# dayae1204/WeCLIP-ViT-CoMer

Hardware: AMD Instinct MI355X
Metric: images/sec (train fwd+bwd) ViT-B/16 512x512 VOC (higher is better)
Workload: dtype f16 MFMA operands / f32 accumulate, f32 residual+softmax+LN, PAR f32 arithmetic on 16-bit fixed-point affinities (precision=fast); 1 GPU; WeCLIP VOC full train step (the reference's model: frozen CLIP ViT-B/16 + adapters + decoder + GradCAM/affinity/PAR pseudo-labels), batch 16/GPU at 512x512, K=2 classes/image (BASELINE configs[2] without the ViT-CoMer inserts, for which the reference has no code); global_batch=16, parallelism=dp1

## Files before the change

### include/weclip_hip.h

```cpp
#ifndef WECLIP_HIP_H
#define WECLIP_HIP_H
#include <stdint.h>
#ifdef __cplusplus
extern "C" {
#endif

int wc_version(void);
const char* wc_last_error(void);
int wc_device_count(void);
int wc_device_arch(int dev, char* buf, int buflen);

void wc_prof_enable(int stride);
void wc_prof_tag(const char* tag);
int wc_prof_report(char* buf, int cap);

int wc_par_affinity(const float* img, float* aff, int B, int H, int W,
                    const int* h_dilations, int n_dil, void* stream);
int wc_par_iterate(const float* aff, const float* masks_in, float* masks_out, int B, int C,
                   int H, int W, const int* h_dilations, int n_dil, void* stream);
int wc_par_forward(const float* img, const float* masks, float* out, float* tmp, float* aff_ws,
                   int B, int C, int H, int W, const int* h_dilations, int n_dil, int num_iter,
                   int group, void* stream);
int wc_par_forward_h(const float* img, const float* masks, float* out, float* tmp, float* aff_ws,
                   int B, int C, int H, int W, const int* h_dilations, int n_dil, int num_iter,
// ... 24 lines not shown
                const void* W2, int nseg, int M, int N, int K, long lda, long ldw, int batch,
                long sA, long sW, long sC, const float* bias, const float* resid, long ldr, long sR,
                float* C32,
                void* C16, void* C16lo, long ldc, int act, int round16, float scale,
                int scale_cols, float* P32, const float* aux, const int* rowmap, int rpg,
                long ldaux, const void* auxh, const float* cscale, long sCS, void* stream);

int wc_gemm_f16_grouped(const void* A0, const void* A1, const void* A2, const void* W0, const void* W1,
                        const void* W2, int nseg, int M, int N, int K, long lda, long ldw, int batch,
                        long sA, long sW, long sC, const float* bias, const float* resid, long ldr, long sR,
                        float* C32, void* C16, void* C16lo, long ldc, int act, int round16, float scale,
                        int scale_cols, float* P32, const float* aux, const int* rowmap, int rpg,
                        long ldaux, const void* auxh, const float* cscale, long sCS, int zdiv, long sA2, long sW2,
                        long sC2, long sB2, long sX2, void* stream);

int wc_gemm_row_supported(int M, int N, int K);
int wc_gemm_row_f16(const void* A, long lda, const void* W, long ldw, int M, int N, int K, const float* bias,
                    const float* cscale, int act, const float* aux, const void* auxh, long ldaux, const float* resid, long ldr,
                    float* C32, void* C16, float* P32, long ldc, long ldc16, const float* ln_g0, const float* ln_b0, void* ln_o0,
                    const float* ln_g1, const float* ln_b1, void* ln_o1, float eps, void* stream);

int wc_gemm_row_f16_grouped(const void* A, long lda, const void* W, long ldw, int M, int N, int K, const float* bias, int act,
                            const void* auxh, long ldaux, float* C32, void* C16, long ldc, long ldc16, int groups, long gA,
                            long gW, long gB, long gC, long gX, void* stream);

int wc_gemm_plan(int M, int N, int K, int nseg, int batch);
int wc_gemm_log_report(char* buf, int cap);
int wc_sum_slices(const float* part, float* out, int nslices, long n, float alpha, void* stream);

int wc_sum_slices_wb(const float* part, float* out_w, float* out_b, int nslices, int rows, int cols,
// ... 24 lines not shown

int wc_attn_fwd(const void* qkv, void* out, float* out32, float* lse, int B, int L, int H, int DH,
                void* stream);
int wc_attn_mean(const void* qkv, const float* lse, float* mean, int B, int L, int H, int DH,
                 void* stream);

int wc_patchify(const float* img, void* hi, void* lo, int B, int H, int W, int P, void* stream);
int wc_cls_rows(float* x, const float* cls, const float* pos0, int B, int L, int E, void* stream);

int wc_cam_head(const float* x2, const float* lnw, const float* lnb, const float* proj,
                const float* text, const int* text_idx, const int* n_text, const int* pair_img,
                const int* pair_cls, float logit_scale, float* partial, float* probs, float* df,
                int B, int P, int L, int E, int Ed, int Tmax, void* stream);
int wc_lnpost_bwd(const float* df, const float* x2, const float* lnw, float gs, const int* pair_img,
                  float* d32, void* dhi, void* dlo, int P, int L, int E, void* stream);
int wc_ln2_bwd_add(const float* da2, const float* dx2, const float* x1, const float* lnw, float gs,
                   const int* pair_img, void* g16, int P, int L, int E, void* stream);
int wc_attn_bwd_colsum(const void* qkv, const void* dO, const float* o32, const float* lse,
                       const int* pair_img, float* delta, float* u, float* dS0, float* P0, float* c,
                       int P, int L, int H, int DH, void* stream);
int wc_rowvec_matmul(const float* c, const float* W, float* out, float* ws, int P, int N, int E, float scale,
                     void* stream);
int wc_cam_map(const float* a32, const float* w, const int* pair_img, float* cam, int P, int L, int E,
               void* stream);

int wc_aff_weight(const float* const* h_maps, int nmaps, const float* wgt, const float* seg, float* W,
                  int B, int L, void* stream);
int wc_aff_seg_weights(const float* const* h_maps, int nmaps, const float* seg, float* diff, float* wgt,
                       int B, int L, void* stream);
int wc_matvec(const float* W, const float* X, const float* sin, const float* sout, const float* add,
// ... 215 lines not shown
```

### weclip-vit-comer_amd/csrc/gemm.hip

```cpp
#include "common.h"
#include <cstring>
#include <stdlib.h>

#include <map>
#include <string>
#include <vector>

struct GemmShapeRec { char key[96]; hipEvent_t e0, e1; double flop; };
static int g_shape_log = -1;
static std::vector<GemmShapeRec> g_shape_recs;
int shape_log_begin(void* stream) {
    if (g_shape_log < 0) g_shape_log = getenv("WECLIP_GEMM_LOG") ? atoi(getenv("WECLIP_GEMM_LOG")) : 0;
    if (!g_shape_log) return -1;
    GemmShapeRec r;
    r.key[0] = 0; r.flop = 0;
    hipEventCreate(&r.e0); hipEventCreate(&r.e1);
    hipEventRecord(r.e0, (hipStream_t)stream);
    g_shape_recs.push_back(r);
    return (int)g_shape_recs.size() - 1;
}
void shape_log_end(int idx, const char* kind, int M, int N, int K, int nseg, int batch, int plan, int act, void* stream) {
    if (idx < 0) return;
    GemmShapeRec& r = g_shape_recs[idx];
    snprintf(r.key, sizeof(r.key), "%s M=%d N=%d K=%d seg=%d batch=%d plan=%d act=%d", kind, M, N, K, nseg, batch, plan, act);
// ... 493 lines not shown
    const long gx = wc_cdiv(N, 256), gy = wc_cdiv(M, 256);
    if (!pp_mode || batch != 1 || (long)K * nseg < 2 * BK || gx * gy < pp_min_tiles) return 0;
    if ((long)M * lda * 2 >= (1L << 32) || (long)N * ldw * 2 >= (1L << 32)) return 0;
    const int n_cu = gemm_cu_count();
    const bool can_split = M % 256 != 0 && !row_mapped_aux;
    const bool split = can_split && wc_cdiv(gx * (gy - 1), n_cu) < wc_cdiv(gx * gy, n_cu);
    return split ? 2 : 1;
}

extern "C" int wc_gemm_plan(int M, int N, int K, int nseg, int batch) {
    return gemm_plan(M, N, K, nseg, batch, false);
}

struct GemmKernel { void (*fn)(GemmArgs); int threads; int lds; const char* name; };
#define GEMM_KERNEL(threads_, lds_, ...) {__VA_ARGS__, threads_, lds_, #__VA_ARGS__}
static const GemmKernel gemm_pp_kernels[4] = {
    GEMM_KERNEL(512, 10 * PP_SLOT, gemm_f16_pp_kernel<0, 10>), GEMM_KERNEL(512, 10 * PP_SLOT, gemm_f16_pp_kernel<1, 10>),
    GEMM_KERNEL(512, 8 * PP_SLOT, gemm_f16_pp_kernel<2, 8>), GEMM_KERNEL(512, 8 * PP_SLOT, gemm_f16_pp_kernel<3, 8>)};
static const GemmKernel gemm_skinny_kernels[4] = {
    GEMM_KERNEL(256, 0, gemm_skinny_kernel<0>), GEMM_KERNEL(256, 0, gemm_skinny_kernel<1>),
    GEMM_KERNEL(256, 0, gemm_skinny_kernel<2>), GEMM_KERNEL(256, 0, gemm_skinny_kernel<3>)};
static const GemmKernel gemm_tile_kernels[2][4] = {
    {GEMM_KERNEL(256, 2 * 2 * BM * BK * 2, gemm_f16_kernel<0, 2>), GEMM_KERNEL(256, 2 * 2 * BM * BK * 2, gemm_f16_kernel<1, 2>),
     GEMM_KERNEL(256, 2 * 2 * BM * BK * 2, gemm_f16_kernel<2, 2>), GEMM_KERNEL(256, 2 * 2 * BM * BK * 2, gemm_f16_kernel<3, 2>)},
    {GEMM_KERNEL(256, 4 * 2 * BM * BK * 2, gemm_f16_kernel<0, 4>), GEMM_KERNEL(256, 4 * 2 * BM * BK * 2, gemm_f16_kernel<1, 4>),
     GEMM_KERNEL(256, 4 * 2 * BM * BK * 2, gemm_f16_kernel<2, 4>), GEMM_KERNEL(256, 4 * 2 * BM * BK * 2, gemm_f16_kernel<3, 4>)}};
#undef GEMM_KERNEL

static bool gemm_reserve_lds(const GemmKernel* k, int n) {
    for (int i = 0; i < n; ++i)
        if (k[i].lds > 65536 &&
            hipFuncSetAttribute((const void*)k[i].fn, hipFuncAttributeMaxDynamicSharedMemorySize, k[i].lds) != hipSuccess)
            return false;
    return true;
}

static int gemm_launch(const GemmKernel& k, const char* family, dim3 grid, const GemmArgs& g, double flop, void* stream) {
    const int pr = wc_prof_begin(stream);
    hipLaunchKernelGGL(k.fn, grid, dim3(k.threads), k.lds, (hipStream_t)stream, g);
    wc_prof_end(pr, k.name, flop, stream);
    WC_LAUNCH_CHECK(family);
    return WC_OK;
}

static int gemm_dispatch(GemmArgs g, int batch, void* stream) {
    int M = g.M;
    const int N = g.N, K = g.K, act = g.act;
    const int ek = ((act == 6 || act == 7) ? 2 : 0) | ((act == 4 || act == 5 || act == 7) ? 1 : 0);
    const int plan = gemm_plan(M, N, K, g.nseg, batch, false, g.lda, g.ldw);
    if (plan) {
        g.gx = wc_cdiv(N, 256);
        g.gy = wc_cdiv(M, 256);
        static bool lds_attr_set = false;
        if (!lds_attr_set) {
            WC_CHECK_ARG(gemm_reserve_lds(gemm_pp_kernels, 4), "wc_gemm_f16: cannot reserve 160 KiB of LDS");
            lds_attr_set = true;
        }
        const int m_main = M / 256 * 256, m_rem = M - m_main;
        const bool split = plan == 2;
        if (split) {
            g.M = m_main;
            g.gy -= 1;
        }
        const dim3 gridp((unsigned)(g.gx * (g.gy >= 16 ? (g.gy + 7) / 8 * 8 : g.gy)), 1, 1);
        const int rc = gemm_launch(gemm_pp_kernels[ek], "gemm_f16_pp_kernel", gridp, g, 2.0 * g.M * N * K, stream);
        if (rc != WC_OK || !split) return rc;
        for (int i = 0; i < g.nseg; ++i) g.A[i] += (long)m_main * g.lda;
        if (g.resid) g.resid += (long)m_main * g.ldr;
        if (g.C32) g.C32 += (long)m_main * g.ldc;
        if (g.C16) g.C16 += (long)m_main * g.ldc;
        if (g.C16lo) g.C16lo += (long)m_main * g.ldc;
        if (g.P32) g.P32 += (long)m_main * g.ldc;
        if (g.aux && !g.rowmap) g.aux += (long)m_main * g.ldaux;
        if (g.rowmap) g.row0 = m_main;
        if (g.auxh) g.auxh += (long)m_main * g.ldaux;
        g.M = M = m_rem;
    }
    if (M <= 32 && batch == 1 && N >= 256)
        return gemm_launch(gemm_skinny_kernels[ek], "gemm_skinny_kernel", dim3(wc_cdiv(N, 64)), g, 2.0 * M * N * K, stream);
    g.gx = wc_cdiv(N, BN);
    g.gy = wc_cdiv(M, BM);
    const dim3 grid((unsigned)(g.gx * ((g.gy + 7) / 8 * 8)), 1, batch);
    static bool lds_attr_set128 = false;
    if (!lds_attr_set128) {
        WC_CHECK_ARG(gemm_reserve_lds(gemm_tile_kernels[1], 4), "wc_gemm_f16: cannot reserve 128 KiB of LDS");
        lds_attr_set128 = true;
    }
    const bool ring = (long)g.gx * g.gy * batch <= gemm_cu_count() && K / BK * g.nseg >= 3;
    return gemm_launch(gemm_tile_kernels[ring][ek], "gemm_f16_kernel", grid, g, 2.0 * g.M * N * K * batch, stream);
}

extern "C" int wc_gemm_f16_grouped(const void* A0, const void* A1, const void* A2, const void* W0, const void* W1,
                                   const void* W2, int nseg, int M, int N, int K, long lda, long ldw, int batch, long sA,
                                   long sW, long sC, const float* bias, const float* resid, long ldr, long sR, float* C32,
                                   void* C16, void* C16lo, long ldc, int act, int round16, float scale, int scale_cols,
                                   float* P32, const float* aux, const int* rowmap, int rpg, long ldaux, const void* auxh,
                                   const float* cscale, long sCS, int zdiv, long sA2, long sW2, long sC2, long sB2,
                                   long sX2, void* stream) {
    const int sl = shape_log_begin(stream);
    WC_CHECK_ARG(zdiv >= 1 && sA2 % 8 == 0 && sW2 % 8 == 0, "wc_gemm_f16_grouped: zdiv >= 1, sA2 / sW2 %% 8 == 0");
// ... 29 lines not shown
    return rc;
}

extern "C" int wc_gemm_f16(const void* A0, const void* A1, const void* A2, const void* W0,
                           const void* W1, const void* W2, int nseg, int M, int N, int K, long lda,
                           long ldw, int batch, long sA, long sW, long sC, const float* bias,
                           const float* resid, long ldr, long sR, float* C32, void* C16, void* C16lo, long ldc, int act,
                           int round16, float scale, int scale_cols, float* P32, const float* aux,
                           const int* rowmap, int rpg, long ldaux, const void* auxh, const float* cscale,
                           long sCS, void* stream) {
    return wc_gemm_f16_grouped(A0, A1, A2, W0, W1, W2, nseg, M, N, K, lda, ldw, batch, sA, sW, sC, bias, resid, ldr, sR,
                               C32, C16, C16lo, ldc, act, round16, scale, scale_cols, P32, aux, rowmap, rpg, ldaux, auxh,
                               cscale, sCS, batch, 0, 0, 0, 0, 0, stream);
}

__global__ __launch_bounds__(256) void split_f16_kernel(const float* __restrict__ x,
                                                         __half* __restrict__ hi,
                                                         __half* __restrict__ lo, long n) {
    long i = ((long)blockIdx.x * 256 + threadIdx.x) * 4;
    const long stride = (long)gridDim.x * 256 * 4;
    for (; i + 3 < n; i += stride) {
        const float4 v = *reinterpret_cast<const float4*>(x + i);
        const float f[4] = {v.x, v.y, v.z, v.w};
        __half h[4], l[4];
#pragma unroll
        for (int k = 0; k < 4; ++k) {
            h[k] = __float2half(f[k]);
            l[k] = __float2half(f[k] - __half2float(h[k]));
        }
        *reinterpret_cast<uint2*>(hi + i) = *reinterpret_cast<uint2*>(h);
// ... 22 lines not shown
```

### weclip-vit-comer_amd/csrc/gemm_common.h

```cpp
#pragma once
#include "common.h"

int shape_log_begin(void* stream);
void shape_log_end(int idx, const char* kind, int M, int N, int K, int nseg, int batch, int plan, int act, void* stream);

static inline int gemm_cu_count() {
    static int n_cu = 0;
    if (!n_cu) {
        int dev = 0;
        if (hipGetDevice(&dev) != hipSuccess ||
            hipDeviceGetAttribute(&n_cu, hipDeviceAttributeMultiprocessorCount, dev) != hipSuccess || n_cu <= 0)
            n_cu = 256;
    }
    return n_cu;
}

typedef _Float16 f16x8 __attribute__((ext_vector_type(8)));
typedef float f32x16 __attribute__((ext_vector_type(16)));
typedef float f32x4 __attribute__((ext_vector_type(4)));

#define BM 128
#define BN 128
#define BK 64

// ... 17 lines not shown
    int scale_cols;
    float* P32;
    const float* aux;
    const int* rowmap;
    int row0;
    int rpg;
    long ldaux;
    const __half* auxh;
    const float* cscale;
    long sCS;
    int gx, gy;
    int auxvec;
    int vec;
    int zdiv;
    long sA2, sW2, sC2, sB2, sX2;
};

#define WC_EPI_ACT(v_, n_)                                                                        \
    if (act == 1) {                                                                               \
        _Pragma("unroll") for (int e_ = 0; e_ < (n_); ++e_)                                       \
            (v_)[e_] = (v_)[e_] * __builtin_amdgcn_rcpf(1.0f + __expf(-1.702f * (v_)[e_]));                   \
    } else if (act == 2) {                                                                        \
        _Pragma("unroll") for (int e_ = 0; e_ < (n_); ++e_) (v_)[e_] = fmaxf((v_)[e_], 0.f);      \
    } else if (act == 3) {                                                                        \
        _Pragma("unroll") for (int e_ = 0; e_ < (n_); ++e_) (v_)[e_] = __builtin_amdgcn_rcpf(1.0f + __expf(-(v_)[e_])); \
    } else if (ERF && act == 6) {       \
        _Pragma("unroll") for (int e_ = 0; e_ < (n_); ++e_)                                       \
            (v_)[e_] = wc_gelu((v_)[e_]);                                                                  \
    }

__device__ __forceinline__ void gemm_colvals(const GemmArgs& g, int n0, int wc, int lane, long zb, float (&bv)[2],
                                             float (&sc)[2], long bbase = 0) {
#pragma unroll
    for (int ni = 0; ni < 2; ++ni) {
        const int col = n0 + wc * 64 + ni * 32 + (lane & 31);
        const int colc = col < g.N ? col : g.N - 1;
        bv[ni] = g.bias ? g.bias[bbase + colc] : 0.f;
        sc[ni] = (col < g.scale_cols) ? g.scale : 1.0f;
        if (g.cscale) sc[ni] *= g.cscale[zb * g.sCS + colc];
    }
}

template <int EK>
__device__ __forceinline__ void gemm_epilogue(const GemmArgs& g, const f32x16 (&acc)[2][2], int m0, int n0, int wr, int wc,
                                              int lane, long zb, char* scratch, const float (&bv)[2],
                                              const float (&sc)[2], long cb, long xb = 0) {
    constexpr bool AUX = (EK & 1) != 0, ERF = EK >= 2;
    const int act = g.act;
    const int rowl = 4 * (lane >> 5);
#define EPI_ROWC(r_) (((r_) & 3) + 8 * (((r_) >> 2) & 3))
#define EPI_ROW(r_) (rowl + EPI_ROWC(r_))
#define EPI_COL(ni_) ((ni_) * 32 + (lane & 31))
    const bool has_res = g.resid != nullptr;
    const bool r16 = g.round16 != 0;
    if (g.vec && !g.P32 && g.C16 && !g.C32) {
        float* tile0 = reinterpret_cast<float*>(scratch);
        const int c4 = (lane & 15) * 4;
        const int gcol = n0 + wc * 64 + c4;
        const bool full = gcol + 3 < g.N;
        const bool has_lo = g.C16lo != nullptr;
        const bool has_sc = g.scale_cols > 0 || g.cscale != nullptr;
        float ua[2][4][4];
// ... 247 lines not shown
```

### weclip-vit-comer_amd/csrc/gradcam.hip

```cpp
#include "common.h"

typedef _Float16 f16x8 __attribute__((ext_vector_type(8)));
typedef float f32x16 __attribute__((ext_vector_type(16)));

#define LNP_ROWS 16
template <int NV>
__global__ __launch_bounds__(256) void lnpost_pool_kernel(const float* __restrict__ x2,
                                                           const float* __restrict__ w,
                                                           const float* __restrict__ bb, float eps,
                                                           float* __restrict__ partial, int L, int E,
                                                           int nchunk) {
    extern __shared__ float sm[];
    const int b = blockIdx.y, chunk = blockIdx.x, lane = threadIdx.x & 63, wv = threadIdx.x >> 6;
    float acc[NV], wv_[NV], bv[NV];
#pragma unroll
    for (int i = 0; i < NV; ++i) {
        const int e = lane + 64 * i;
        acc[i] = 0.f;
        wv_[i] = e < E ? w[e] : 0.f;
        bv[i] = e < E ? bb[e] : 0.f;
    }
    const int l0 = chunk * LNP_ROWS;
    for (int l = l0 + wv; l < l0 + LNP_ROWS && l < L; l += 4) {
        if (l == 0) continue;
// ... 133 lines not shown
            s += __shfl_xor(s, 1, 64);
            s += __shfl_xor(s, 2, 64);
            s += __shfl_xor(s, 4, 64);
            if (j == 0 && e < E) df[(long)p * E + e] = s;
        }
    } else {
        for (int e = tid; e < E; e += 512) {
            const float* pr = proj + (long)e * Ed;
            float s = 0.f;
            for (int k = 0; k < Ed; ++k) s = fmaf(pr[k], dy[k], s);
            df[(long)p * E + e] = s;
        }
    }
}

template <int NV>
__global__ __launch_bounds__(256) void lnpost_bwd_kernel(const float* __restrict__ df,
                                                          const float* __restrict__ x2,
                                                          const float* __restrict__ w, float eps, float gs,
                                                          const int* __restrict__ pair_img,
                                                          float* __restrict__ d32, __half* __restrict__ dhi,
                                                          __half* __restrict__ dlo, int L, int E, long rows) {
    const long row = (long)blockIdx.x * 4 + (threadIdx.x >> 6);
    if (row >= rows) return;
    const int lane = threadIdx.x & 63;
    const int p = row / L, l = row % L;
    const long o = row * E;
    if (l == 0) {
        for (int e = lane; e < E; e += 64) {
            d32[o + e] = 0.f;
            dhi[o + e] = __float2half(0.f);
            if (dlo) dlo[o + e] = __float2half(0.f);
        }
        return;
    }
    const float* xr = x2 + ((long)pair_img[p] * L + l) * E;
    const float* g0 = df + (long)p * E;
    const float invn = 1.0f / (L - 1);
    if constexpr (NV > 0) {
        float xv[NV], gv[NV];
        float s = 0.f;
#pragma unroll
        for (int i = 0; i < NV; ++i) {
            const int e = lane + 64 * i, ec = e < E ? e : 0;
            const float ok = e < E ? 1.f : 0.f;
            xv[i] = xr[ec] * ok;
            gv[i] = g0[ec] * invn * w[ec] * ok;
            s += xv[i];
        }
        const float mean = wave_sum(s) / E;
        float q = 0.f;
// ... 5 lines not shown
        const float rstd = rsqrtf(wave_sum(q) / E + eps);
        float sg = 0.f, sgx = 0.f;
#pragma unroll
        for (int i = 0; i < NV; ++i) {
            sg += gv[i];
            sgx += gv[i] * (xv[i] - mean) * rstd;
        }
        sg = wave_sum(sg) / E;
        sgx = wave_sum(sgx) / E;
#pragma unroll
        for (int i = 0; i < NV; ++i) {
            const int e = lane + 64 * i;
            if (e < E) {
                const float v = gs * rstd * (gv[i] - sg - (xv[i] - mean) * rstd * sgx);
                d32[o + e] = v;
                const __half h = __float2half(v);
                dhi[o + e] = h;
                if (dlo) dlo[o + e] = __float2half(v - __half2float(h));
            }
        }
    } else {
        float s = 0.f;
        for (int e = lane; e < E; e += 64) s += xr[e];
        const float mean = wave_sum(s) / E;
        float q = 0.f;
        for (int e = lane; e < E; e += 64) { const float d = xr[e] - mean; q += d * d; }
        const float rstd = rsqrtf(wave_sum(q) / E + eps);
        float sg = 0.f, sgx = 0.f;
        for (int e = lane; e < E; e += 64) {
            const float g = g0[e] * invn * w[e];
            sg += g;
            sgx += g * (xr[e] - mean) * rstd;
        }
        sg = wave_sum(sg) / E;
        sgx = wave_sum(sgx) / E;
        for (int e = lane; e < E; e += 64) {
            const float g = g0[e] * invn * w[e];
            const float v = gs * rstd * (g - sg - (xr[e] - mean) * rstd * sgx);
            d32[o + e] = v;
            const __half h = __float2half(v);
            dhi[o + e] = h;
            if (dlo) dlo[o + e] = __float2half(v - __half2float(h));
        }
    }
}

template <int NV>
__global__ __launch_bounds__(256) void ln2_bwd_add_kernel(const float* __restrict__ da2,
                                                           const float* __restrict__ dx2,
                                                           const float* __restrict__ x1,
                                                           const float* __restrict__ w, float eps,
                                                           float inv_gs, const int* __restrict__ pair_img,
                                                           __half* __restrict__ g16, int L, int E, long rows) {
    const long row = (long)blockIdx.x * 4 + (threadIdx.x >> 6);
    if (row >= rows) return;
    const int lane = threadIdx.x & 63;
    const int p = row / L, l = row % L;
// ... 389 lines not shown
    const size_t sm = (E + 2 * Ed + Tmax + 16) * sizeof(float);
    hipLaunchKernelGGL(cam_head_kernel, dim3(P), dim3(512), sm, st, partial, proj, text, text_idx, n_text,
                       pair_img, pair_cls, logit_scale, probs, df, L, E, Ed, nchunk, Tmax);
    WC_LAUNCH_CHECK("cam_head_kernel");
    return WC_OK;
}

extern "C" int wc_lnpost_bwd(const float* df, const float* x2, const float* lnw, float gs,
                             const int* pair_img, float* d32, void* dhi, void* dlo, int P, int L, int E,
                             void* stream) {
    WC_CHECK_ARG(df && x2 && lnw && pair_img && d32 && dhi && P > 0 && L > 1 && E > 0,
                 "wc_lnpost_bwd: bad argument");
    const long rows = (long)P * L;
#define LNPOST_BWD(NV_)                                                                                            \
    hipLaunchKernelGGL(lnpost_bwd_kernel<NV_>, dim3(wc_cdiv(rows, 4)), dim3(256), 0, (hipStream_t)stream, df, x2, \
                       lnw, 1e-5f, gs, pair_img, d32, (__half*)dhi, (__half*)dlo, L, E, rows)
    if (E <= 256) LNPOST_BWD(4);
    else if (E <= 768) LNPOST_BWD(12);
    else if (E <= 1024) LNPOST_BWD(16);
    else LNPOST_BWD(0);
#undef LNPOST_BWD
    WC_LAUNCH_CHECK("lnpost_bwd_kernel");
    return WC_OK;
}

extern "C" int wc_ln2_bwd_add(const float* da2, const float* dx2, const float* x1, const float* lnw, float gs,
                              const int* pair_img, void* g16, int P, int L, int E, void* stream) {
    WC_CHECK_ARG(da2 && dx2 && x1 && lnw && pair_img && g16 && P > 0 && L > 0 && E > 0 && gs > 0,
                 "wc_ln2_bwd_add: bad argument");
    const long rows = (long)P * L;
    WC_CHECK_ARG(E <= 1024, "wc_ln2_bwd_add: E <= 1024");
// ... 130 lines not shown
```

### weclip-vit-comer_amd/gradcam_engine.py

```python
import torch

from . import _lib as L
from . import ops
from .ops import F16, F32, Split
from .clip import vit_engine as VE

def _logit_scale(clip_model):
    p = clip_model.logit_scale
    key = (p.data_ptr(), p._version)
    cached = getattr(clip_model, "_logit_scale_host", None)
    if cached is None or cached[0] != key:
        cached = (key, float(p.detach().exp().item()))
        clip_model._logit_scale_host = cached
    return cached[1]


GRAD_SCALE = 4096.0


class _BwdPack:

    def __init__(self, blk):
        t = lambda w: ops.split_f16(w.detach().float().t().contiguous())
        self.pjT = t(blk.mlp.c_proj.weight)
        self.fcT = t(blk.mlp.c_fc.weight)
        self.outT = t(blk.attn.out_proj.weight)
        self.w_in = blk.attn.in_proj_weight.detach().float().contiguous()
        self.ln2_w = blk.ln_2.weight.detach().float().contiguous()


class LastLayerState:

    def __init__(self, clip_model, x2, mean, keep, B, Lq):
        self.m, self.x2, self.mean, self.keep, self.B, self.L = clip_model, x2, mean, keep, B, Lq
        blk = clip_model.visual.transformer.resblocks[-1]
        if getattr(blk, "_bwd_pack", None) is None or blk._bwd_pack.w_in.device != x2.device:
            blk._bwd_pack = _BwdPack(blk)
        self.bw = blk._bwd_pack
        self.blk = blk
# ... 32 lines not shown
        lib = L.lib()
        k, bw = self.keep, self.bw
        B, Lq = self.B, self.L
        E = self.x2.shape[1]
        H = self.blk.attn.num_heads
        DH = E // H
        P = pair_img.numel()
        M = P * Lq
        dev = self.x2.device
        st = L.stream
        probs, df = self._head(text_hat, text_idx, n_text, pair_img, pair_cls, Tmax)
        v = self.m.visual
        dx2 = torch.empty(M, E, device=dev, dtype=F32)
        from . import config
        ex = config.exact()
        dx2s = Split(torch.empty(M, E, device=dev, dtype=F16), torch.empty(M, E, device=dev, dtype=F16) if ex else None)
        lib.wc_lnpost_bwd(L.ptr(df), L.ptr(self.x2), L.ptr(v.ln_post.weight.detach().float(), F32),
                          GRAD_SCALE, L.ptr(pair_img), L.ptr(dx2), L.ptr(dx2s.hi), L.ptr(dx2s.lo), P, Lq, E,
                          st())
        du = Split(torch.empty(M, 4 * E, device=dev, dtype=F16), torch.empty(M, 4 * E, device=dev, dtype=F16) if ex else None)
        ops.gemm(dx2s, bw.pjT, M, 4 * E, E, out16=du.hi, out16lo=du.lo, act=4, aux=k["u32"],
                 rowmap=pair_img, rpg=Lq, ldaux=4 * E)
        da2 = torch.empty(M, E, device=dev, dtype=F32)
        ops.gemm(du, bw.fcT, M, E, 4 * E, out32=da2)
        g16 = torch.empty(M, E, device=dev, dtype=F16)
        lib.wc_ln2_bwd_add(L.ptr(da2), L.ptr(dx2), L.ptr(k["x1"]), L.ptr(bw.ln2_w), GRAD_SCALE,
                           L.ptr(pair_img), L.ptr(g16), P, Lq, E, st())
        do16 = torch.empty(M, E, device=dev, dtype=F16)
        ops.gemm(g16, bw.outT, M, E, E, out16=do16)
        ws = torch.empty(4, P, H, Lq, device=dev, dtype=F32)
        c = torch.empty(P, 3 * E, device=dev, dtype=F32)
        lib.wc_attn_bwd_colsum(L.ptr(k["qkv"]), L.ptr(do16), L.ptr(k["o32"]), L.ptr(k["lse"]),
                               L.ptr(pair_img), L.ptr(ws[0]), L.ptr(ws[1]), L.ptr(ws[2]), L.ptr(ws[3]),
                               L.ptr(c), P, Lq, H, DH, st())
        w = torch.empty(P, E, device=dev, dtype=F32)
        ws2 = torch.empty(16 * P * E, device=dev, dtype=F32)
        lib.wc_rowvec_matmul(L.ptr(c), L.ptr(bw.w_in), L.ptr(w), L.ptr(ws2), P, 3 * E, E, 1.0 / (Lq - 1), st())
# ... 11 lines not shown
```

### weclip-vit-comer_amd/ops.py

```python
import ctypes
import math

import torch

from . import _lib as L

F16 = torch.float16
F32 = torch.float32
LOG2E = 1.4426950408889634


class KernelTimer:

    active = False

    @staticmethod
    def enable(stride=1):
        L.lib().cdll.wc_prof_enable(int(stride))
        KernelTimer.active = bool(stride)
        if not stride:
            L.lib().cdll.wc_prof_tag(None)

    @staticmethod
    def tag(name):
# ... 42 lines not shown
    lda = K if lda is None else lda
    ldw = K if ldw is None else ldw
    ldc = N if ldc is None else ldc
    ap = [L.ptr(s[0], F16, "A") for s in segs] + [None] * (3 - len(segs))
    wp = [L.ptr(s[1], F16, "W") for s in segs] + [None] * (3 - len(segs))
    ldr = ldc if ldr is None else ldr
    sR = sC if sR is None else sR
    L.lib().wc_gemm_f16_grouped(ap[0], ap[1], ap[2], wp[0], wp[1], wp[2], len(segs), M, N, K, lda, ldw,
                                batch, sA, sW, sC, L.ptr(bias, F32, "bias"), L.ptr(resid, F32, "resid"),
                                ldr, sR, L.ptr(out32, F32, "out32"), L.ptr(out16, F16, "out16"),
                                L.ptr(out16lo, F16, "out16lo"), ldc, act, 1 if round16 else 0,
                                float(scale), scale_cols, L.ptr(pre32, F32, "pre32"), L.ptr(aux, F32, "aux"),
                                L.ptr(rowmap, torch.int32, "rowmap"), rpg, ldaux, L.ptr(auxh, F16, "auxh"),
                                L.ptr(cscale, F32, "cscale"), sCS, batch if zdiv is None else zdiv, sA2, sW2, sC2, sB2,
                                sX2, L.stream())


def gemm_row_ok(M, N, K):
    return N <= 256 and N % 4 == 0 and K in (128, 256) and M > 0


def gemm_row(a16, w16, M, N, K, *, lda=None, ldw=None, bias=None, cscale=None, act=0, aux=None, auxh=None, ldaux=0, resid=None,
             ldr=None, out32=None, out16=None, pre32=None, ldc=None, ldc16=None, ln=(), eps=1e-5):
    lda = K if lda is None else lda
    ldw = K if ldw is None else ldw
    ldc = N if ldc is None else ldc
    ldr = ldc if ldr is None else ldr
    ldc16 = ldc if ldc16 is None else ldc16
    lnp = [None] * 6
    for i, (gam, bet, out) in enumerate(ln):
# ... 288 lines not shown
```

Before: 1303 images/sec.

## Share GradCAM backward c_proj GEMM across class pairs of the same image

The GradCAM backward through the last block's MLP previously ran the c_proj-transpose GEMM on every (image,class) pair's LN-post gradient, i.e. P*L rows. The ln_post backward gradient is now decomposed algebraically into a per-image normalized input (shared by all pairs of that image) plus per-pair rank-one corrections. The GEMM therefore runs once per image (B*L rows), and a new epilogue expands each output row to all pairs of that image using a pair table, per-pair scalars and a small per-pair row-vector product. This roughly halves the GEMM work when K=2 classes per image, at the cost of a more complex epilogue with indirect loads and scattered stores, plus an extra single-block table kernel and a rowvec matmul.

```diff
diff --git a/include/weclip_hip.h b/include/weclip_hip.h
--- a/include/weclip_hip.h
+++ b/include/weclip_hip.h
@@ -62,6 +62,11 @@
                         long ldaux, const void* auxh, const float* cscale, long sCS, int zdiv, long sA2, long sW2,
                         long sC2, long sB2, long sX2, void* stream);
 
+int wc_gemm_f16_pairs(const void* A0, const void* A1, const void* A2, const void* W0, const void* W1, const void* W2,
+                      int nseg, int M, int N, int K, long lda, long ldw, const float* aux, long ldaux, int rpg, int nimg,
+                      const float* rs, const float* s, const float* c, const int* first, const int* list, float scale,
+                      void* C16, void* C16lo, long ldc, void* stream);
+
 int wc_gemm_row_supported(int M, int N, int K);
 int wc_gemm_row_f16(const void* A, long lda, const void* W, long ldw, int M, int N, int K, const float* bias,
                     const float* cscale, int act, const float* aux, const void* auxh, long ldaux, const float* resid, long ldr,
@@ -116,6 +121,9 @@
                 int B, int P, int L, int E, int Ed, int Tmax, void* stream);
 int wc_lnpost_bwd(const float* df, const float* x2, const float* lnw, float gs, const int* pair_img,
                   float* d32, void* dhi, void* dlo, int P, int L, int E, void* stream);
+int wc_lnpost_bwd_shared(const float* df, const float* x2, const float* lnw, float gs, const int* pair_img, float* d32,
+                         void* xhi, void* xlo, float* rs, float* s, float* hc, int* first, int* list, int* pos, int B, int P,
+                         int L, int E, void* stream);
 int wc_ln2_bwd_add(const float* da2, const float* dx2, const float* x1, const float* lnw, float gs,
                    const int* pair_img, void* g16, int P, int L, int E, void* stream);
 int wc_attn_bwd_colsum(const void* qkv, const void* dO, const float* o32, const float* lse,
diff --git a/weclip-vit-comer_amd/csrc/gemm.hip b/weclip-vit-comer_amd/csrc/gemm.hip
--- a/weclip-vit-comer_amd/csrc/gemm.hip
+++ b/weclip-vit-comer_amd/csrc/gemm.hip
@@ -531,17 +531,21 @@
 
 struct GemmKernel { void (*fn)(GemmArgs); int threads; int lds; const char* name; };
 #define GEMM_KERNEL(threads_, lds_, ...) {__VA_ARGS__, threads_, lds_, #__VA_ARGS__}
-static const GemmKernel gemm_pp_kernels[4] = {
+static const GemmKernel gemm_pp_kernels[5] = {
     GEMM_KERNEL(512, 10 * PP_SLOT, gemm_f16_pp_kernel<0, 10>), GEMM_KERNEL(512, 10 * PP_SLOT, gemm_f16_pp_kernel<1, 10>),
-    GEMM_KERNEL(512, 8 * PP_SLOT, gemm_f16_pp_kernel<2, 8>), GEMM_KERNEL(512, 8 * PP_SLOT, gemm_f16_pp_kernel<3, 8>)};
-static const GemmKernel gemm_skinny_kernels[4] = {
+    GEMM_KERNEL(512, 8 * PP_SLOT, gemm_f16_pp_kernel<2, 8>), GEMM_KERNEL(512, 8 * PP_SLOT, gemm_f16_pp_kernel<3, 8>),
+    GEMM_KERNEL(512, 10 * PP_SLOT, gemm_f16_pp_kernel<4, 10>)};
+static const GemmKernel gemm_skinny_kernels[5] = {
     GEMM_KERNEL(256, 0, gemm_skinny_kernel<0>), GEMM_KERNEL(256, 0, gemm_skinny_kernel<1>),
-    GEMM_KERNEL(256, 0, gemm_skinny_kernel<2>), GEMM_KERNEL(256, 0, gemm_skinny_kernel<3>)};
-static const GemmKernel gemm_tile_kernels[2][4] = {
+    GEMM_KERNEL(256, 0, gemm_skinny_kernel<2>), GEMM_KERNEL(256, 0, gemm_skinny_kernel<3>),
+    GEMM_KERNEL(256, 0, gemm_skinny_kernel<4>)};
+static const GemmKernel gemm_tile_kernels[2][5] = {
     {GEMM_KERNEL(256, 2 * 2 * BM * BK * 2, gemm_f16_kernel<0, 2>), GEMM_KERNEL(256, 2 * 2 * BM * BK * 2, gemm_f16_kernel<1, 2>),
-     GEMM_KERNEL(256, 2 * 2 * BM * BK * 2, gemm_f16_kernel<2, 2>), GEMM_KERNEL(256, 2 * 2 * BM * BK * 2, gemm_f16_kernel<3, 2>)},
+     GEMM_KERNEL(256, 2 * 2 * BM * BK * 2, gemm_f16_kernel<2, 2>), GEMM_KERNEL(256, 2 * 2 * BM * BK * 2, gemm_f16_kernel<3, 2>),
+     GEMM_KERNEL(256, 2 * 2 * BM * BK * 2, gemm_f16_kernel<4, 2>)},
     {GEMM_KERNEL(256, 4 * 2 * BM * BK * 2, gemm_f16_kernel<0, 4>), GEMM_KERNEL(256, 4 * 2 * BM * BK * 2, gemm_f16_kernel<1, 4>),
-     GEMM_KERNEL(256, 4 * 2 * BM * BK * 2, gemm_f16_kernel<2, 4>), GEMM_KERNEL(256, 4 * 2 * BM * BK * 2, gemm_f16_kernel<3, 4>)}};
+     GEMM_KERNEL(256, 4 * 2 * BM * BK * 2, gemm_f16_kernel<2, 4>), GEMM_KERNEL(256, 4 * 2 * BM * BK * 2, gemm_f16_kernel<3, 4>),
+     GEMM_KERNEL(256, 4 * 2 * BM * BK * 2, gemm_f16_kernel<4, 4>)}};
 #undef GEMM_KERNEL
 
 static bool gemm_reserve_lds(const GemmKernel* k, int n) {
@@ -563,14 +567,14 @@
 static int gemm_dispatch(GemmArgs g, int batch, void* stream) {
     int M = g.M;
     const int N = g.N, K = g.K, act = g.act;
-    const int ek = ((act == 6 || act == 7) ? 2 : 0) | ((act == 4 || act == 5 || act == 7) ? 1 : 0);
+    const int ek = act == 8 ? 4 : ((act == 6 || act == 7) ? 2 : 0) | ((act == 4 || act == 5 || act == 7) ? 1 : 0);
     const int plan = gemm_plan(M, N, K, g.nseg, batch, false, g.lda, g.ldw);
     if (plan) {
         g.gx = wc_cdiv(N, 256);
         g.gy = wc_cdiv(M, 256);
         static bool lds_attr_set = false;
         if (!lds_attr_set) {
-            WC_CHECK_ARG(gemm_reserve_lds(gemm_pp_kernels, 4), "wc_gemm_f16: cannot reserve 160 KiB of LDS");
+            WC_CHECK_ARG(gemm_reserve_lds(gemm_pp_kernels, 5), "wc_gemm_f16: cannot reserve 160 KiB of LDS");
             lds_attr_set = true;
         }
         const int m_main = M / 256 * 256, m_rem = M - m_main;
@@ -585,11 +589,12 @@
         for (int i = 0; i < g.nseg; ++i) g.A[i] += (long)m_main * g.lda;
         if (g.resid) g.resid += (long)m_main * g.ldr;
         if (g.C32) g.C32 += (long)m_main * g.ldc;
-        if (g.C16) g.C16 += (long)m_main * g.ldc;
-        if (g.C16lo) g.C16lo += (long)m_main * g.ldc;
+        const bool pairs = act == 8;
+        if (g.C16 && !pairs) g.C16 += (long)m_main * g.ldc;
+        if (g.C16lo && !pairs) g.C16lo += (long)m_main * g.ldc;
         if (g.P32) g.P32 += (long)m_main * g.ldc;
-        if (g.aux && !g.rowmap) g.aux += (long)m_main * g.ldaux;
-        if (g.rowmap) g.row0 = m_main;
+        if (g.aux && !g.rowmap && !pairs) g.aux += (long)m_main * g.ldaux;
+        if (g.rowmap || pairs) g.row0 = m_main;
         if (g.auxh) g.auxh += (long)m_main * g.ldaux;
         g.M = M = m_rem;
     }
@@ -600,7 +605,7 @@
     const dim3 grid((unsigned)(g.gx * ((g.gy + 7) / 8 * 8)), 1, batch);
     static bool lds_attr_set128 = false;
     if (!lds_attr_set128) {
-        WC_CHECK_ARG(gemm_reserve_lds(gemm_tile_kernels[1], 4), "wc_gemm_f16: cannot reserve 128 KiB of LDS");
+        WC_CHECK_ARG(gemm_reserve_lds(gemm_tile_kernels[1], 5), "wc_gemm_f16: cannot reserve 128 KiB of LDS");
         lds_attr_set128 = true;
     }
     const bool ring = (long)g.gx * g.gy * batch <= gemm_cu_count() && K / BK * g.nseg >= 3;
@@ -660,6 +665,34 @@
                                cscale, sCS, batch, 0, 0, 0, 0, 0, stream);
 }
 
+extern "C" int wc_gemm_f16_pairs(const void* A0, const void* A1, const void* A2, const void* W0, const void* W1, const void* W2,
+                                 int nseg, int M, int N, int K, long lda, long ldw, const float* aux, long ldaux, int rpg,
+                                 int nimg, const float* rs, const float* s, const float* c, const int* first, const int* list,
+                                 float scale, void* C16, void* C16lo, long ldc, void* stream) {
+    const int sl = shape_log_begin(stream);
+    WC_CHECK_ARG(nseg >= 1 && nseg <= 3, "wc_gemm_f16_pairs: nseg must be 1..3");
+    WC_CHECK_ARG(M > 0 && N > 0 && K > 0 && K % BK == 0, "wc_gemm_f16_pairs: need M,N>0 and K %% 64 == 0 (got M=%d N=%d K=%d)", M, N, K);
+    WC_CHECK_ARG(A0 && W0 && (nseg < 2 || (A1 && W1)) && (nseg < 3 || (A2 && W2)), "wc_gemm_f16_pairs: null operand");
+    WC_CHECK_ARG(lda % 8 == 0 && ldw % 8 == 0 && lda >= K && ldw >= K, "wc_gemm_f16_pairs: operand rows must be 16-byte aligned");
+    WC_CHECK_ARG(((uintptr_t)A0 | (uintptr_t)W0 | (uintptr_t)A1 | (uintptr_t)W1 | (uintptr_t)A2 | (uintptr_t)W2) % 16 == 0,
+                 "wc_gemm_f16_pairs: operands must be 16-byte aligned");
+    WC_CHECK_ARG(aux && rs && s && c && first && list && C16, "wc_gemm_f16_pairs: null side input or output");
+    WC_CHECK_ARG(rpg > 0 && nimg > 0 && (long)nimg * rpg == M, "wc_gemm_f16_pairs: M must be nimg * rpg");
+    WC_CHECK_ARG(N % 4 == 0 && ldc % 4 == 0 && ldc >= N && ldaux % 4 == 0 && ldaux >= N && (uintptr_t)aux % 16 == 0 &&
+                     (uintptr_t)c % 16 == 0 && (uintptr_t)C16 % 8 == 0 && (uintptr_t)C16lo % 8 == 0,
+                 "wc_gemm_f16_pairs: N, ldc, ldaux %% 4 == 0; aux, c 16-byte and outputs 8-byte aligned");
+    GemmArgs g = {};
+    g.A[0] = (const __half*)A0; g.A[1] = (const __half*)A1; g.A[2] = (const __half*)A2;
+    g.W[0] = (const __half*)W0; g.W[1] = (const __half*)W1; g.W[2] = (const __half*)W2;
+    g.nseg = nseg; g.M = M; g.N = N; g.K = K; g.lda = lda; g.ldw = ldw;
+    g.C16 = (__half*)C16; g.C16lo = (__half*)C16lo; g.ldc = ldc;
+    g.act = 8; g.scale = scale; g.aux = aux; g.rpg = rpg; g.ldaux = ldaux; g.vec = 1; g.zdiv = 1;
+    g.prs = rs; g.ps = s; g.pc = c; g.pfirst = first; g.plist = list;
+    const int rc = gemm_dispatch(g, 1, stream);
+    if (sl >= 0) shape_log_end(sl, "f16", M, N, K, nseg, 1, gemm_plan(M, N, K, nseg, 1, false, lda, ldw), 8, stream);
+    return rc;
+}
+
 __global__ __launch_bounds__(256) void split_f16_kernel(const float* __restrict__ x,
                                                          __half* __restrict__ hi,
                                                          __half* __restrict__ lo, long n) {
diff --git a/weclip-vit-comer_amd/csrc/gemm_common.h b/weclip-vit-comer_amd/csrc/gemm_common.h
--- a/weclip-vit-comer_amd/csrc/gemm_common.h
+++ b/weclip-vit-comer_amd/csrc/gemm_common.h
@@ -55,6 +55,11 @@
     int vec;
     int zdiv;
     long sA2, sW2, sC2, sB2, sX2;
+    const float* prs;
+    const float* ps;
+    const float* pc;
+    const int* pfirst;
+    const int* plist;
 };
 
 #define WC_EPI_ACT(v_, n_)                                                                        \
@@ -82,11 +87,114 @@
     }
 }
 
+__device__ __forceinline__ void gemm_epilogue_pairs(const GemmArgs& g, const f32x16 (&acc)[2][2], int m0, int n0, int wr, int wc,
+                                                    int lane, char* scratch) {
+    float* tile0 = reinterpret_cast<float*>(scratch);
+    const int rowl = 4 * (lane >> 5);
+    const int c4 = (lane & 15) * 4;
+    const int gcol = n0 + wc * 64 + c4;
+    const bool colok = gcol < g.N;
+    const int gcolc = colok ? gcol : 0;
+    const bool has_lo = g.C16lo != nullptr;
+    float4 ua[2][4];
+    int beg[2][4], cnt[2][4];
+    auto row_of = [&](int c, int it, int& arow, int& img) {
+        const int grow = m0 + wr * 64 + c * 16 + it * 4 + (lane >> 4);
+        arow = (grow < g.M ? grow : g.M - 1) + g.row0;
+        img = arow / g.rpg;
+        return grow < g.M && colok;
+    };
+    auto side_load = [&](int c, float4 (&u4)[4], int (&bg)[4], int (&cn)[4]) {
+        int arow[4], img[4], en[4];
+        bool ok[4];
+#pragma unroll
+        for (int it = 0; it < 4; ++it) ok[it] = row_of(c, it, arow[it], img[it]);
+#pragma unroll
+        for (int it = 0; it < 4; ++it) { bg[it] = g.pfirst[img[it]]; en[it] = g.pfirst[img[it] + 1]; }
+#pragma unroll
+        for (int it = 0; it < 4; ++it) u4[it] = *reinterpret_cast<const float4*>(g.aux + (long)arow[it] * g.ldaux + gcolc);
+#pragma unroll
+        for (int it = 0; it < 4; ++it) cn[it] = ok[it] ? en[it] - bg[it] : 0;
+    };
+    side_load(0, ua[0], beg[0], cnt[0]);
+#pragma unroll
+    for (int c = 0; c < 4; ++c) {
+        const int mi = c >> 1, rq0 = (c & 1) * 8, sb = c & 1;
+        float* tile = tile0 + sb * 1024;
+        if (c + 1 < 4) side_load(c + 1, ua[sb ^ 1], beg[sb ^ 1], cnt[sb ^ 1]);
+        int tok[4];
+        float rsv[4];
+#pragma unroll
+        for (int it = 0; it < 4; ++it) {
+            int arow, img;
+            row_of(c, it, arow, img);
+            tok[it] = arow - img * g.rpg;
+            rsv[it] = g.prs[arow];
+        }
+#pragma unroll
+        for (int ni = 0; ni < 2; ++ni)
+#pragma unroll
+            for (int rr = 0; rr < 8; ++rr)
+                tile[(rowl + (rr & 3) + 8 * (rr >> 2)) * 64 + ni * 32 + (lane & 31)] = acc[mi][ni][rq0 + rr];
+        float f[4][4], gd[4][4];
+        int cmax = 0;
+#pragma unroll
+        for (int it = 0; it < 4; ++it) {
+            const float4 t4 = *reinterpret_cast<const float4*>(tile + (it * 4 + (lane >> 4)) * 64 + c4);
+            f[it][0] = t4.x; f[it][1] = t4.y; f[it][2] = t4.z; f[it][3] = t4.w;
+            const float uu[4] = {ua[sb][it].x, ua[sb][it].y, ua[sb][it].z, ua[sb][it].w};
+            const float rg = g.scale * rsv[it];
+#pragma unroll
+            for (int k = 0; k < 4; ++k) {
+                const float sg = __builtin_amdgcn_rcpf(1.0f + __expf(-1.702f * uu[k]));
+                gd[it][k] = rg * (sg * (1.0f + 1.702f * uu[k] * (1.0f - sg)));
+            }
+            cmax = cnt[sb][it] > cmax ? cnt[sb][it] : cmax;
+        }
+        for (int k = 0; __any(k < cmax); ++k) {
+            int j[4], pr[4];
+            float sv[4];
+            float4 cv[4];
+#pragma unroll
+            for (int it = 0; it < 4; ++it) {
+                const int kk = k < cnt[sb][it] ? k : cnt[sb][it] - 1;
+                j[it] = beg[sb][it] + kk > 0 ? beg[sb][it] + kk : 0;
+            }
+#pragma unroll
+            for (int it = 0; it < 4; ++it) pr[it] = g.plist[j[it]];
+#pragma unroll
+            for (int it = 0; it < 4; ++it) sv[it] = g.ps[(long)j[it] * g.rpg + tok[it]];
+#pragma unroll
+            for (int it = 0; it < 4; ++it) cv[it] = *reinterpret_cast<const float4*>(g.pc + (long)j[it] * g.N + gcolc);
+#pragma unroll
+            for (int it = 0; it < 4; ++it) {
+                const float v[4] = {(cv[it].x - sv[it] * f[it][0]) * gd[it][0], (cv[it].y - sv[it] * f[it][1]) * gd[it][1],
+                                    (cv[it].z - sv[it] * f[it][2]) * gd[it][2], (cv[it].w - sv[it] * f[it][3]) * gd[it][3]};
+                __half h[4], l[4];
+#pragma unroll
+                for (int e = 0; e < 4; ++e) {
+                    h[e] = __float2half(v[e]);
+                    l[e] = __float2half(v[e] - __half2float(h[e]));
+                }
+                if (k < cnt[sb][it]) {
+                    const long o = ((long)pr[it] * g.rpg + tok[it]) * g.ldc + gcol;
+                    __builtin_nontemporal_store(*reinterpret_cast<u32x2*>(h), reinterpret_cast<u32x2*>(g.C16 + o));
+                    if (has_lo) __builtin_nontemporal_store(*reinterpret_cast<u32x2*>(l), reinterpret_cast<u32x2*>(g.C16lo + o));
+                }
+            }
+        }
+    }
+}
+
 template <int EK>
 __device__ __forceinline__ void gemm_epilogue(const GemmArgs& g, const f32x16 (&acc)[2][2], int m0, int n0, int wr, int wc,
                                               int lane, long zb, char* scratch, const float (&bv)[2],
                                               const float (&sc)[2], long cb, long xb = 0) {
-    constexpr bool AUX = (EK & 1) != 0, ERF = EK >= 2;
+    if constexpr (EK == 4) {
+        gemm_epilogue_pairs(g, acc, m0, n0, wr, wc, lane, scratch);
+        return;
+    }
+    constexpr bool AUX = (EK & 1) != 0, ERF = EK == 2 || EK == 3;
     const int act = g.act;
     const int rowl = 4 * (lane >> 5);
 #define EPI_ROWC(r_) (((r_) & 3) + 8 * (((r_) >> 2) & 3))
diff --git a/weclip-vit-comer_amd/csrc/gradcam.hip b/weclip-vit-comer_amd/csrc/gradcam.hip
--- a/weclip-vit-comer_amd/csrc/gradcam.hip
+++ b/weclip-vit-comer_amd/csrc/gradcam.hip
@@ -171,27 +171,83 @@
     }
 }
 
-template <int NV>
+__global__ __launch_bounds__(256) void pair_table_kernel(const int* __restrict__ pair_img, int* __restrict__ first,
+                                                          int* __restrict__ list, int* __restrict__ pos, int B, int P) {
+    extern __shared__ int cur[];
+    for (int b = threadIdx.x; b < B; b += 256) {
+        int n = 0;
+        for (int p = 0; p < P; ++p) n += pair_img[p] == b ? 1 : 0;
+        cur[b] = n;
+    }
+    __syncthreads();
+    if (threadIdx.x == 0) {
+        int a = 0;
+        for (int b = 0; b < B; ++b) {
+            const int n = cur[b];
+            cur[b] = a;
+            first[b] = a;
+            a += n;
+        }
+        first[B] = a;
+    }
+    __syncthreads();
+    for (int b = threadIdx.x; b < B; b += 256) {
+        int j = cur[b];
+        for (int p = 0; p < P; ++p)
+            if (pair_img[p] == b) {
+                list[j] = p;
+                pos[p] = j;
+                ++j;
+            }
+    }
+}
+
+template <int NV, bool SH = false>
 __global__ __launch_bounds__(256) void lnpost_bwd_kernel(const float* __restrict__ df,
                                                           const float* __restrict__ x2,
                                                           const float* __restrict__ w, float eps, float gs,
                                                           const int* __restrict__ pair_img,
                                                           float* __restrict__ d32, __half* __restrict__ dhi,
-                                                          __half* __restrict__ dlo, int L, int E, long rows) {
+                                                          __half* __restrict__ dlo, int L, int E, long rows,
+                                                          float* __restrict__ rs = nullptr, float* __restrict__ sc = nullptr,
+                                                          float* __restrict__ hc = nullptr, const int* __restrict__ first = nullptr,
+                                                          const int* __restrict__ pos = nullptr) {
     const long row = (long)blockIdx.x * 4 + (threadIdx.x >> 6);
     if (row >= rows) return;
     const int lane = threadIdx.x & 63;
     const int p = row / L, l = row % L;
     const long o = row * E;
+    const int img = pair_img[p];
+    int slot = 0;
+    bool lead = false;
+    long ox = 0;
+    if constexpr (SH) {
+        slot = pos[p];
+        lead = first[img] == slot;
+        ox = ((long)img * L + l) * E;
+    }
     if (l == 0) {
         for (int e = lane; e < E; e += 64) {
             d32[o + e] = 0.f;
-            dhi[o + e] = __float2half(0.f);
-            if (dlo) dlo[o + e] = __float2half(0.f);
+            if constexpr (SH) {
+                if (lead) {
+                    dhi[ox + e] = __float2half(0.f);
+                    if (dlo) dlo[ox + e] = __float2half(0.f);
+                }
+            } else {
+                dhi[o + e] = __float2half(0.f);
+                if (dlo) dlo[o + e] = __float2half(0.f);
+            }
+        }
+        if constexpr (SH) {
+            if (lane == 0) {
+                sc[(long)slot * L] = 0.f;
+                if (lead) rs[(long)img * L] = 0.f;
+            }
         }
         return;
     }
-    const float* xr = x2 + ((long)pair_img[p] * L + l) * E;
+    const float* xr = x2 + ((long)img * L + l) * E;
     const float* g0 = df + (long)p * E;
     const float invn = 1.0f / (L - 1);
     if constexpr (NV > 0) {
@@ -227,9 +283,25 @@
             if (e < E) {
                 const float v = gs * rstd * (gv[i] - sg - (xv[i] - mean) * rstd * sgx);
                 d32[o + e] = v;
-                const __half h = __float2half(v);
-                dhi[o + e] = h;
-                if (dlo) dlo[o + e] = __float2half(v - __half2float(h));
+                if constexpr (SH) {
+                    if (l == 1) hc[(long)slot * E + e] = gv[i] - sg;
+                    if (lead) {
+                        const float xn = (xv[i] - mean) * rstd;
+                        const __half h = __float2half(xn);
+                        dhi[ox + e] = h;
+                        if (dlo) dlo[ox + e] = __float2half(xn - __half2float(h));
+                    }
+                } else {
+                    const __half h = __float2half(v);
+                    dhi[o + e] = h;
+                    if (dlo) dlo[o + e] = __float2half(v - __half2float(h));
+                }
+            }
+        }
+        if constexpr (SH) {
+            if (lane == 0) {
+                sc[(long)slot * L + l] = sgx;
+                if (lead) rs[(long)img * L + l] = rstd;
             }
         }
     } else {
@@ -251,9 +323,25 @@
             const float g = g0[e] * invn * w[e];
             const float v = gs * rstd * (g - sg - (xr[e] - mean) * rstd * sgx);
             d32[o + e] = v;
-            const __half h = __float2half(v);
-            dhi[o + e] = h;
-            if (dlo) dlo[o + e] = __float2half(v - __half2float(h));
+            if constexpr (SH) {
+                if (l == 1) hc[(long)slot * E + e] = g - sg;
+                if (lead) {
+                    const float xn = (xr[e] - mean) * rstd;
+                    const __half h = __float2half(xn);
+                    dhi[ox + e] = h;
+                    if (dlo) dlo[ox + e] = __float2half(xn - __half2float(h));
+                }
+            } else {
+                const __half h = __float2half(v);
+                dhi[o + e] = h;
+                if (dlo) dlo[o + e] = __float2half(v - __half2float(h));
+            }
+        }
+        if constexpr (SH) {
+            if (lane == 0) {
+                sc[(long)slot * L + l] = sgx;
+                if (lead) rs[(long)img * L + l] = rstd;
+            }
         }
     }
 }
@@ -673,7 +761,31 @@
     const long rows = (long)P * L;
 #define LNPOST_BWD(NV_)                                                                                            \
     hipLaunchKernelGGL(lnpost_bwd_kernel<NV_>, dim3(wc_cdiv(rows, 4)), dim3(256), 0, (hipStream_t)stream, df, x2, \
-                       lnw, 1e-5f, gs, pair_img, d32, (__half*)dhi, (__half*)dlo, L, E, rows)
+                       lnw, 1e-5f, gs, pair_img, d32, (__half*)dhi, (__half*)dlo, L, E, rows, (float*)nullptr,     \
+                       (float*)nullptr, (float*)nullptr, (const int*)nullptr, (const int*)nullptr)
+    if (E <= 256) LNPOST_BWD(4);
+    else if (E <= 768) LNPOST_BWD(12);
+    else if (E <= 1024) LNPOST_BWD(16);
+    else LNPOST_BWD(0);
+#undef LNPOST_BWD
+    WC_LAUNCH_CHECK("lnpost_bwd_kernel");
+    return WC_OK;
+}
+
+extern "C" int wc_lnpost_bwd_shared(const float* df, const float* x2, const float* lnw, float gs, const int* pair_img,
+                                    float* d32, void* xhi, void* xlo, float* rs, float* s, float* hc, int* first, int* list,
+                                    int* pos, int B, int P, int L, int E, void* stream) {
+    WC_CHECK_ARG(df && x2 && lnw && pair_img && d32 && xhi && rs && s && hc && first && list && pos && B > 0 && P > 0 &&
+                     L > 1 && E > 0, "wc_lnpost_bwd_shared: bad argument");
+    WC_CHECK_ARG(B <= 8192, "wc_lnpost_bwd_shared: B <= 8192");
+    hipLaunchKernelGGL(pair_table_kernel, dim3(1), dim3(256), B * sizeof(int), (hipStream_t)stream, pair_img, first, list, pos,
+                       B, P);
+    WC_LAUNCH_CHECK("pair_table_kernel");
+    const long rows = (long)P * L;
+#define LNPOST_BWD(NV_)                                                                                                  \
+    hipLaunchKernelGGL((lnpost_bwd_kernel<NV_, true>), dim3(wc_cdiv(rows, 4)), dim3(256), 0, (hipStream_t)stream, df, x2, \
+                       lnw, 1e-5f, gs, pair_img, d32, (__half*)xhi, (__half*)xlo, L, E, rows, rs, s, hc,                 \
+                       (const int*)first, (const int*)pos)
     if (E <= 256) LNPOST_BWD(4);
     else if (E <= 768) LNPOST_BWD(12);
     else if (E <= 1024) LNPOST_BWD(16);
diff --git a/weclip-vit-comer_amd/gradcam_engine.py b/weclip-vit-comer_amd/gradcam_engine.py
--- a/weclip-vit-comer_amd/gradcam_engine.py
+++ b/weclip-vit-comer_amd/gradcam_engine.py
@@ -23,6 +23,7 @@
     def __init__(self, blk):
         t = lambda w: ops.split_f16(w.detach().float().t().contiguous())
         self.pjT = t(blk.mlp.c_proj.weight)
+        self.pj32 = blk.mlp.c_proj.weight.detach().float().contiguous()
         self.fcT = t(blk.mlp.c_fc.weight)
         self.outT = t(blk.attn.out_proj.weight)
         self.w_in = blk.attn.in_proj_weight.detach().float().contiguous()
@@ -85,13 +86,21 @@
         dx2 = torch.empty(M, E, device=dev, dtype=F32)
         from . import config
         ex = config.exact()
-        dx2s = Split(torch.empty(M, E, device=dev, dtype=F16), torch.empty(M, E, device=dev, dtype=F16) if ex else None)
-        lib.wc_lnpost_bwd(L.ptr(df), L.ptr(self.x2), L.ptr(v.ln_post.weight.detach().float(), F32),
-                          GRAD_SCALE, L.ptr(pair_img), L.ptr(dx2), L.ptr(dx2s.hi), L.ptr(dx2s.lo), P, Lq, E,
-                          st())
+        xn = Split(torch.empty(B * Lq, E, device=dev, dtype=F16), torch.empty(B * Lq, E, device=dev, dtype=F16) if ex else None)
+        rs = torch.empty(B * Lq, device=dev, dtype=F32)
+        sc = torch.empty(P * Lq, device=dev, dtype=F32)
+        hc = torch.empty(P, E, device=dev, dtype=F32)
+        tab = torch.empty(B + 1 + 2 * P, device=dev, dtype=torch.int32)
+        first, plist, pos = tab[:B + 1], tab[B + 1:B + 1 + P], tab[B + 1 + P:]
+        lib.wc_lnpost_bwd_shared(L.ptr(df), L.ptr(self.x2), L.ptr(v.ln_post.weight.detach().float(), F32), GRAD_SCALE,
+                                 L.ptr(pair_img), L.ptr(dx2), L.ptr(xn.hi), L.ptr(xn.lo), L.ptr(rs), L.ptr(sc), L.ptr(hc),
+                                 L.ptr(first), L.ptr(plist), L.ptr(pos), B, P, Lq, E, st())
+        cp = torch.empty(P, 4 * E, device=dev, dtype=F32)
+        ws1 = torch.empty(16 * P * 4 * E, device=dev, dtype=F32)
+        lib.wc_rowvec_matmul(L.ptr(hc), L.ptr(bw.pj32), L.ptr(cp), L.ptr(ws1), P, E, 4 * E, 1.0, st())
         du = Split(torch.empty(M, 4 * E, device=dev, dtype=F16), torch.empty(M, 4 * E, device=dev, dtype=F16) if ex else None)
-        ops.gemm(dx2s, bw.pjT, M, 4 * E, E, out16=du.hi, out16lo=du.lo, act=4, aux=k["u32"],
-                 rowmap=pair_img, rpg=Lq, ldaux=4 * E)
+        ops.gemm_pairs(xn, bw.pjT, B * Lq, 4 * E, E, aux=k["u32"], ldaux=4 * E, rpg=Lq, nimg=B, rs=rs, s=sc, c=cp,
+                       first=first, plist=plist, scale=GRAD_SCALE, out16=du.hi, out16lo=du.lo)
         da2 = torch.empty(M, E, device=dev, dtype=F32)
         ops.gemm(du, bw.fcT, M, E, 4 * E, out32=da2)
         g16 = torch.empty(M, E, device=dev, dtype=F16)
diff --git a/weclip-vit-comer_amd/ops.py b/weclip-vit-comer_amd/ops.py
--- a/weclip-vit-comer_amd/ops.py
+++ b/weclip-vit-comer_amd/ops.py
@@ -80,6 +80,23 @@
                                 L.ptr(rowmap, torch.int32, "rowmap"), rpg, ldaux, L.ptr(auxh, F16, "auxh"),
                                 L.ptr(cscale, F32, "cscale"), sCS, batch if zdiv is None else zdiv, sA2, sW2, sC2, sB2,
                                 sX2, L.stream())
+
+
+def gemm_pairs(a, w, M, N, K, *, aux, ldaux, rpg, nimg, rs, s, c, first, plist, scale, out16, out16lo=None, ldc=None):
+    a = a if isinstance(a, Split) else Split(a)
+    w = w if isinstance(w, Split) else Split(w)
+    segs = [(a.hi, w.hi)]
+    if a.lo is not None:
+        segs.append((a.lo, w.hi))
+    if w.lo is not None:
+        segs.append((a.hi, w.lo))
+    ap = [L.ptr(x[0], F16, "A") for x in segs] + [None] * (3 - len(segs))
+    wp = [L.ptr(x[1], F16, "W") for x in segs] + [None] * (3 - len(segs))
+    L.lib().wc_gemm_f16_pairs(ap[0], ap[1], ap[2], wp[0], wp[1], wp[2], len(segs), M, N, K, K, K, L.ptr(aux, F32, "aux"),
+                              ldaux, rpg, nimg, L.ptr(rs, F32, "rs"), L.ptr(s, F32, "s"), L.ptr(c, F32, "c"),
+                              L.ptr(first, torch.int32, "first"), L.ptr(plist, torch.int32, "plist"), float(scale),
+                              L.ptr(out16, F16, "out16"), L.ptr(out16lo, F16, "out16lo"), N if ldc is None else ldc,
+                              L.stream())
 
 
 def gemm_row_ok(M, N, K):
```

Result: no change. 1313 images/sec (median of 6 runs) (+0.8%).
